# Jiawei-Yang/Denoising-ViT

Measured on AMD Instinct MI355X. Metric: stage-1 images denoised/sec (DINOv2-B/14, 518px, 1k Adam steps), higher is better.
Workload: dtype bf16

## Files before the change

### denoising-vit_amd/csrc/dvt_vit.hip

```cpp
#include <math.h>

#include <type_traits>

#include "../../include/dvt_vit.h"
#include "dvt_common.h"
#include "dvt_ln_row.h"

typedef short bf16x8 __attribute__((ext_vector_type(8)));
typedef short bf16x4 __attribute__((ext_vector_type(4)));
typedef float f32x4 __attribute__((ext_vector_type(4)));
typedef unsigned short bf16_t;

extern int g_f32x3_exact_attention, g_f32x3_unfused;

namespace {

typedef __bf16 hw_bf16x2 __attribute__((ext_vector_type(2)));
typedef float f32x2 __attribute__((ext_vector_type(2)));

__device__ __forceinline__ uint32_t pack2(float a, float b) {
  const hw_bf16x2 v = __builtin_convertvector((f32x2){a, b}, hw_bf16x2);
  return __builtin_bit_cast(uint32_t, v);
}
__device__ __forceinline__ bf16_t f2bf(float f) { return (bf16_t)(pack2(f, 0.f) & 0xffffu); }

constexpr int GBM = 128, GBN = 128, GBK = 64;
int g_vit_gemm_variant = 4;
constexpr int STAGE_BYTES = (GBM + GBN) * GBK * 2;

enum { EPI_BIAS = 0, EPI_QKV = 1, EPI_GELU = 2, EPI_RESID = 3, EPI_EMBED = 4, EPI_F32 = 5, EPI_GELU_X3 = 6, EPI_QKV_X3 = 7,
       EPI_SWIGLU = 8 };
#define IS_QKV(E) ((E) == EPI_QKV || (E) == EPI_QKV_X3)
#define IS_GELU(E) ((E) == EPI_GELU || (E) == EPI_GELU_X3)
#define IS_X3(E) ((E) == EPI_GELU_X3 || (E) == EPI_QKV_X3)

#include "dvt_tile_map.h"

enum { EPOL_RESID_LD = 1,
       EPOL_RESID_ST = 2,
       EPOL_XB_ST = 4,
       EPOL_HID_ST = 8,
       EPOL_QKV_ST = 16,
       EPOL_HID_SC1 = 32,
       EPOL_RESID_SC1 = 64,
       EPOL_ALL = 127,
       EPOL_DEFAULT = EPOL_RESID_LD | EPOL_RESID_ST | EPOL_XB_ST | EPOL_HID_ST | EPOL_HID_SC1 };

struct GemmBArgs {
  const bf16_t* A;
  const bf16_t* W;
  int M, N, K;
  const float* bias;
  bf16_t* out;
  bf16_t* vt;
  bf16_t* out_lo;
  bf16_t* vt_lo;
  float* x;
  const float* gamma;
  const float* pos;
  const float* cls;
  int dim, heads, s_pad, n_tokens;
  int n_prefix, pos_has_cls;
  int group;
  int mblock;
  int nt_store;
  const float2* ln_stats;
  const float* ln_cs;
  bf16_t* xb;
  float2* st_part;
// ... 982 lines not shown
  }
}

#ifdef DVT_LAB
#include "lab/dvt_vit_gemm8t.inc"
#endif
#undef P8B_TILE
#undef P8_STAGE
#undef P8_STAGE_RS
#undef P8_RSRC
#undef P8_RD
#undef P8_LANE_SETUP

#ifdef DVT_LAB
typedef const __attribute__((address_space(4))) GemmBArgs* kernarg_ptr_t;

#include "lab/dvt_vit_gemm4w.inc"
#include "lab/dvt_vit_gemm8p_lab.inc"
#include "lab/dvt_vit_lab.inc"
#endif

int g_vit_group_bytes = 4800 * 1024;
int g_vit_mblock = 0;
int g_vit_nt_store = 0;
int g_vit_xcols = 0;
int g_vit_xcols_bytes = 2400 * 1024;
int g_vit_epi_policy = -1;
int g_vit_fuse_ln = 1;
int g_vit_attn_mask = 15;
int g_vit_stagger_pct = 0;
int g_vit_attn_log2q = 1;
constexpr float ATT_Q_PRESCALE = 0.125f * 1.4426950408889634f;
int g_vit_pf_next = 0;
constexpr int ATT_L2_VAR = 559;
#ifdef DVT_LAB
int g_vit_tpw = 0;
int g_vit_attn_l2_mask = ATT_L2_VAR;
int g_vit_epi_abl = 0;
int g_vit_attn_variant = 2;
int g_vit_abl4w = 0;
int g_vit_8p_build = 0;
unsigned* g_vit_dbg = nullptr;
int g_vit_w4_grid = 0;
#endif

template <int EPI>
int launch_gemm(const GemmBArgs& a0, hipStream_t s) {
  if (a0.M % GBM || a0.N % GBN || a0.K % GBK || a0.M <= 0) return DVT_E_BADARG;
  if (IS_X3(EPI) && a0.M % 256) return DVT_E_BADARG;
  GemmBArgs a = a0;
  if (!a.lda) a.lda = a.K;
  if (!a.ldw) a.ldw = a.K;
  a.dim_ok_sq = (!IS_QKV(EPI)) || (a.dim % 256 == 0);
  if (IS_QKV(EPI) && (a.s_pad <= 0 || a.s_pad % 8 || a.vt_rows <= 0 || a.vt_rows % a.s_pad || a.vt_rows > a.M))
    return DVT_E_BADARG;
  bool sq = g_vit_gemm_variant >= 4;
#ifdef DVT_LAB
  sq = sq || g_vit_gemm_variant == 0;
#endif
  sq = sq && a.M % 256 == 0 && a.N % 256 == 0 && a.dim_ok_sq && a.K >= 2 * GBK && (a.K / GBK) % 2 == 0;
  if (a.ln_stats != nullptr && !(sq || (a.M % G2_BM == 0 && g_vit_gemm_variant != 1))) return DVT_E_BADARG;
  if ((a.xb != nullptr || a.st_part != nullptr) && !(sq && EPI == EPI_RESID && a.xb != nullptr && a.st_part != nullptr))
    return DVT_E_BADARG;
  {
    const int nt = a.N / GBN;
    int g = g_vit_group_bytes / (GBN * a.K * 2);
    g = g < 1 ? 1 : (g > nt ? nt : g);
// ... 260 lines not shown
  const int bb = row / n_tokens, s = row - bb * n_tokens;
  float* y;
  if (s < n_prefix) {
    if (prefix == nullptr) return;
    y = prefix + ((size_t)bb * n_prefix + s) * dim;
  } else {
    y = feat + ((size_t)bb * (n_tokens - n_prefix) + (s - n_prefix)) * dim;
  }
  const float4* xr = reinterpret_cast<const float4*>(x + ((size_t)bb * s_pad + s) * dim);
  const int nq = dim >> 2;
  if (NORM) {
    float4 v[NV];
    float mean, rstd;
    ln_row_stats<NV>(xr, nq, dim, eps, lane, v, mean, rstd);
#pragma unroll
    for (int i = 0; i < NV; ++i) {
      const int q = lane + 64 * i;
      if (q < nq)
        reinterpret_cast<float4*>(y)[q] =
            ln_row_piece(v[i], mean, rstd, reinterpret_cast<const float4*>(w)[q], reinterpret_cast<const float4*>(b)[q]);
    }
  } else {
#pragma unroll
    for (int i = 0; i < NV; ++i) {
      const int q = lane + 64 * i;
      if (q < nq) reinterpret_cast<float4*>(y)[q] = xr[q];
    }
  }
}

__device__ __forceinline__ float max3f(float a, float b, float c) {
  return __builtin_fmaxf(__builtin_fmaxf(a, b), c);
}

constexpr int KV_TILE = 64;
constexpr int VT_LD = 128;

constexpr int ATT_Q = 128;

#ifdef DVT_LAB
#include "lab/dvt_vit_lab_attn.inc"
#endif


constexpr int ATT2_KBUF = 3;

template <int VAR, bool X3>
__device__ __forceinline__ void attention_v2_body(const bf16_t* __restrict__ qk, const bf16_t* __restrict__ vt,
                                                  bf16_t* __restrict__ out, int heads, int s_pad, int n_valid,
                                                  const bf16_t* __restrict__ qk_lo, const bf16_t* __restrict__ vt_lo,
                                                  int split_out = 0) {
  constexpr int NV = (VAR & 64) ? 3 : 2;
  constexpr bool L2D = (VAR & 32) != 0;
  constexpr bool SKIPW = L2D && !(VAR & 128), HALFT = L2D && !(VAR & 256);
  static_assert(!L2D || ((VAR & 4) && !X3 && !(VAR & 64)), "log2-domain build: on the no-max-tree structure, bf16 only");
  constexpr int KBUF = L2D ? 4 : ATT2_KBUF;
  constexpr int KSET = KBUF * KV_TILE * 128, VSET = NV * 64 * VT_LD;
  __shared__ __attribute__((aligned(16))) char smem[(X3 ? 2 : 1) * (KSET + VSET)];
  char* const Kb = smem;
  char* const Vb = smem + KSET;
  char* const Kbl = smem + KSET + VSET;
  char* const Vbl = Kbl + KSET;
  const int tid = threadIdx.x, lane = tid & 63, wave = tid >> 6;
  const int g = lane >> 4, lc = lane & 15;
  const int nqb = (s_pad + ATT_Q - 1) / ATT_Q;
  int id = blockIdx.x;
  {
    const int nwg = gridDim.x, q = nwg >> 3, r = nwg & 7, xcd = id & 7, loc = id >> 3;
    id = (xcd < r ? xcd * (q + 1) : r * (q + 1) + (xcd - r) * q) + loc;
  }
  const int qb = id % nqb, h = (id / nqb) % heads, b = id / (nqb * heads);
  const int dim = heads * 64, ldq = 2 * dim;
  const size_t row0 = (size_t)b * s_pad;

  bf16x8 qf[2], qfl[2];
  auto load_q = [&](const bf16_t* base, bf16x8 (&dst)[2]) {
    const bf16_t* qrow = base + (row0 + qb * ATT_Q + wave * 16 + lc) * ldq + h * 64;
#pragma unroll
    for (int ks = 0; ks < 2; ++ks) {
      union { bf16x8 v; uint32_t u[4]; } raw;
      raw.v = *reinterpret_cast<const bf16x8*>(qrow + ks * 32 + g * 8);
      if constexpr (!L2D) {
#pragma unroll
        for (int j = 0; j < 4; ++j) {
          const float lo = __uint_as_float(raw.u[j] << 16) * 0.125f;
          const float hi = __uint_as_float(raw.u[j] & 0xffff0000u) * 0.125f;
          raw.u[j] = pack2(lo, hi);
        }
      }
      dst[ks] = raw.v;
    }
  };
  load_q(qk, qf);
  if constexpr (X3) load_q(qk_lo, qfl);
  const bf16_t* kbase = qk + row0 * ldq + dim + h * 64;
  const bf16_t* vbase = vt + ((size_t)(b * heads + h) * 64) * s_pad;

  f32x4 o[4];
#pragma unroll
  for (int i = 0; i < 4; ++i) o[i] = (f32x4){0.f, 0.f, 0.f, 0.f};
  float m_run = L2D ? 0.f : -1e30f, l_run = 0.f;
  f32x4 cinit = (f32x4){0.f, 0.f, 0.f, 0.f};
  const f32x4 zero4 = (f32x4){0.f, 0.f, 0.f, 0.f};
  const bool active = !SKIPW || qb * ATT_Q + __builtin_amdgcn_readfirstlane(wave) * 16 < s_pad;
  const float LOG2E = 1.4426950408889634f;
  const float THR = 8.0f;

  const int ntiles = (n_valid + KV_TILE - 1) / KV_TILE;
  const int sr0 = tid >> 3, sc = tid & 7;
  const bf16_t* kp0 = kbase + (size_t)sr0 * ldq + sc * 8;
  const bf16_t* vp0 = vbase + (size_t)sr0 * s_pad + sc * 8;
  const int kdo = sr0 * 128 + ((sc ^ (sr0 & 7)) << 4);
  const int vks = sc >> 2, vc = sc & 3, vsw = (sr0 >> 1) & 7;
  const int vdo0 = sr0 * VT_LD + (((vks * 4 + 2 * (vc & 1)) ^ vsw) << 4) + (vc >> 1) * 8;
  const int vdo1 = sr0 * VT_LD + (((vks * 4 + 2 * (vc & 1) + 1) ^ vsw) << 4) + (vc >> 1) * 8;
  uint4 kr0, vr0, kr0l, vr0l;
  const ptrdiff_t klo = X3 ? (qk_lo - qk) : 0, vlo = X3 ? (vt_lo - vt) : 0;
  const unsigned klane = (unsigned)(sr0 * ldq + sc * 8) * 2u;
  const unsigned vlane = (unsigned)(sr0 * s_pad + sc * 8) * 2u, vlane0 = (unsigned)(sr0 * s_pad) * 2u;
#define A2_LOADK(kt)                                                                                 \
  do {                                                                                               \
    if constexpr (L2D) {                                                                             \
      kr0 = *reinterpret_cast<const uint4*>(reinterpret_cast<const char*>(kbase + (size_t)(kt) * KV_TILE * ldq) + klane); \
    } else {                                                                                         \
      kr0 = *reinterpret_cast<const uint4*>(kp0 + (size_t)(kt) * KV_TILE * ldq);                     \
    }                                                                                                \
    if constexpr (X3) kr0l = *reinterpret_cast<const uint4*>(kp0 + klo + (size_t)(kt) * KV_TILE * ldq); \
  } while (0)
#define A2_LOADV(kt)                                                                   \
  do {                                                                                 \
    if constexpr (L2D) {                                                               \
      const unsigned vo_ = (kt) * KV_TILE + sc * 8 >= s_pad ? vlane0 : vlane;          \
      vr0 = *reinterpret_cast<const uint4*>(reinterpret_cast<const char*>(vbase + (kt) * KV_TILE) + vo_); \
    } else {                                                                           \
      const int vk_ = (kt) * KV_TILE + sc * 8 >= s_pad ? -sc * 8 : (kt) * KV_TILE;     \
      vr0 = *reinterpret_cast<const uint4*>(vp0 + vk_);                                \
      if constexpr (X3) vr0l = *reinterpret_cast<const uint4*>(vp0 + vlo + vk_);       \
    }                                                                                  \
  } while (0)
#define A2_STOREK(kt)                                                                                   \
  do {                                                                                                  \
    *reinterpret_cast<uint4*>(Kb + ((kt) % KBUF) * (KV_TILE * 128) + kdo) = kr0;                   \
    if constexpr (X3) *reinterpret_cast<uint4*>(Kbl + ((kt) % KBUF) * (KV_TILE * 128) + kdo) = kr0l; \
  } while (0)
#define A2_STOREV(kt)                                                                     \
  do {                                                                                    \
    char* vb_ = Vb + ((kt) % NV) * (64 * VT_LD);                                          \
    *reinterpret_cast<uint2*>(vb_ + vdo0) = make_uint2(vr0.x, vr0.y);                     \
    *reinterpret_cast<uint2*>(vb_ + vdo1) = make_uint2(vr0.z, vr0.w);                     \
    if constexpr (X3) {                                                                   \
      char* vl_ = Vbl + ((kt) % NV) * (64 * VT_LD);                                       \
      *reinterpret_cast<uint2*>(vl_ + vdo0) = make_uint2(vr0l.x, vr0l.y);                 \
// ... 11 lines not shown
          const int krow = mt * 16 + lc, ko_ = krow * 128 + (((ks * 4 + g) ^ (krow & 7)) << 4);                     \
          kh_[mt] = *reinterpret_cast<const bf16x8*>(Ks_ + ko_);                                                   \
          kl_[mt] = *reinterpret_cast<const bf16x8*>(Kl_ + ko_);                                                   \
          if (ks == 0) dst[mt] = (f32x4){0.f, 0.f, 0.f, 0.f};                                                      \
        }                                                                                                          \
        _Pragma("unroll") for (int mt = 0; mt < 4; ++mt)                                                           \
          dst[mt] = __builtin_amdgcn_mfma_f32_16x16x32_bf16(kl_[mt], qf[ks], dst[mt], 0, 0, 0);                    \
        _Pragma("unroll") for (int mt = 0; mt < 4; ++mt)                                                           \
          dst[mt] = __builtin_amdgcn_mfma_f32_16x16x32_bf16(kh_[mt], qfl[ks], dst[mt], 0, 0, 0);                   \
        _Pragma("unroll") for (int mt = 0; mt < 4; ++mt)                                                           \
          dst[mt] = __builtin_amdgcn_mfma_f32_16x16x32_bf16(kh_[mt], qf[ks], dst[mt], 0, 0, 0);                    \
      }                                                                                                            \
    } else if constexpr (VAR & 1) {                                                                                       \
      _Pragma("unroll") for (int ks = 0; ks < 2; ++ks) {                                                           \
        _Pragma("unroll") for (int mt = 0; mt < 4; ++mt) {                                                         \
          const int krow = mt * 16 + lc;                                                                           \
          const bf16x8 kf = *reinterpret_cast<const bf16x8*>(Ks_ + krow * 128 + (((ks * 4 + g) ^ (krow & 7)) << 4)); \
          if (ks == 0) dst[mt] = L2D ? cinit : zero4;                                                              \
          dst[mt] = __builtin_amdgcn_mfma_f32_16x16x32_bf16(kf, qf[ks], dst[mt], 0, 0, 0);                         \
        }                                                                                                          \
      }                                                                                                            \
    } else {                                                                                                       \
    _Pragma("unroll") for (int mt = 0; mt < 4; ++mt) {                                                             \
      dst[mt] = L2D ? cinit : zero4;                                                                               \
      _Pragma("unroll") for (int ks = 0; ks < 2; ++ks) {                                                           \
        const int krow = mt * 16 + lc;                                                                             \
        const bf16x8 kf = *reinterpret_cast<const bf16x8*>(Ks_ + krow * 128 + (((ks * 4 + g) ^ (krow & 7)) << 4)); \
        dst[mt] = __builtin_amdgcn_mfma_f32_16x16x32_bf16(kf, qf[ks], dst[mt], 0, 0, 0);                           \
      }                                                                                                            \
    }                                                                                                              \
    }                                                                                                              \
  } while (0)

  A2_LOADK(0);
  A2_LOADV(0);
  A2_STOREK(0);
  A2_STOREV(0);
  if constexpr (L2D) {
    const int last = ntiles - 1;
    A2_LOADK(1 < last ? 1 : last);
    A2_STOREK(1);
    A2_LOADK(2 < last ? 2 : last);
    A2_LOADV(1 < last ? 1 : last);
  } else {
    if (ntiles > 1) {
      A2_LOADK(1);
      A2_STOREK(1);
    }
    if (ntiles > 2) A2_LOADK(2);
    if (ntiles > 1) A2_LOADV(1);
  }
  __syncthreads();
  f32x4 sA[4], sB[4];
  auto lane_quad_max = [&](float v) {
    const unsigned u = __float_as_uint(v);
    const auto r16 = __builtin_amdgcn_permlane16_swap(u, u, false, false);
    v = fmaxf(__uint_as_float(r16[0]), __uint_as_float(r16[1]));
    const unsigned u2 = __float_as_uint(v);
    const auto r32 = __builtin_amdgcn_permlane32_swap(u2, u2, false, false);
    return fmaxf(__uint_as_float(r32[0]), __uint_as_float(r32[1]));
  };
  auto max16 = [&](const f32x4 (&s)[4]) {
    float tmax = __builtin_fmaxf(__builtin_fmaxf(s[0][0], s[0][1]), s[0][2]);
    tmax = max3f(tmax, s[0][3], s[1][0]);
    tmax = max3f(tmax, s[1][1], s[1][2]);
    tmax = max3f(tmax, s[1][3], s[2][0]);
    tmax = max3f(tmax, s[2][1], s[2][2]);
    tmax = max3f(tmax, s[2][3], s[3][0]);
    tmax = max3f(tmax, s[3][1], s[3][2]);
    return fmaxf(tmax, s[3][3]);
  };
  if (active) A2_S(sA, 0);
  if constexpr (L2D) {
    if (active) {
      if (n_valid < KV_TILE) {
#pragma unroll
        for (int mt = 0; mt < 4; ++mt)
#pragma unroll
          for (int r = 0; r < 4; ++r)
            if (mt * 16 + 4 * g + r >= n_valid) sA[mt][r] = -1e30f;
      }
      m_run = lane_quad_max(max16(sA));
      cinit = (f32x4){-m_run, -m_run, -m_run, -m_run};
#pragma unroll
      for (int mt = 0; mt < 4; ++mt) sA[mt] += cinit;
    }
  }
  if constexpr (VAR & 16) {
    if (wave >= 4) __builtin_amdgcn_s_setprio(1);
  }
  if constexpr (VAR & 64) {
    if (wave >= 4) __syncthreads();
  }
  union PF { bf16x8 v; uint32_t u[4]; };
  auto tile = [&](int kt, auto last_tag, f32x4 (&s)[4], f32x4 (&sn)[4]) {
    constexpr bool LAST = decltype(last_tag)::value;
    if constexpr (L2D) {
      const int last = ntiles - 1;
      A2_STOREK(kt + 2);
      A2_STOREV(kt + 1);
      if constexpr (!LAST) {
        const int k3 = kt + 3 < last ? kt + 3 : last, v2 = kt + 2 < last ? kt + 2 : last;
        A2_LOADK(k3);
        A2_LOADV(v2);
      }
    } else {
    if (kt + 2 < ntiles) A2_STOREK(kt + 2);
    if (kt + 1 < ntiles) A2_STOREV(kt + 1);
    if (kt + 3 < ntiles) A2_LOADK(kt + 3);
    if (kt + 2 < ntiles) A2_LOADV(kt + 2);
    }
    if constexpr (LAST) {
      const int kbase_idx = kt * KV_TILE;
#pragma unroll
      for (int mt = 0; mt < 4; ++mt)
#pragma unroll
        for (int r = 0; r < 4; ++r)
          if (kbase_idx + mt * 16 + 4 * g + r >= n_valid) s[mt][r] = -1e30f;
    }
    auto exact_max = [&]() {
      if constexpr (L2D) {
        const float d = fmaxf(lane_quad_max(max16(s)), 0.f);
        const float alpha = __builtin_amdgcn_exp2f(-d);
        l_run *= alpha;
#pragma unroll
        for (int i = 0; i < 4; ++i) o[i] *= alpha;
        m_run += d;
        cinit = (f32x4){-m_run, -m_run, -m_run, -m_run};
        const f32x4 d4 = {d, d, d, d};
#pragma unroll
        for (int mt = 0; mt < 4; ++mt) {
          s[mt] -= d4;
          if constexpr (!LAST) sn[mt] -= d4;
        }
        return;
      }
// ... 35 lines not shown
      if (!__all(tmax <= m_run + THR)) {
        const unsigned u = __float_as_uint(tmax);
        const auto r16 = __builtin_amdgcn_permlane16_swap(u, u, false, false);
        tmax = fmaxf(__uint_as_float(r16[0]), __uint_as_float(r16[1]));
        const unsigned u2 = __float_as_uint(tmax);
        const auto r32 = __builtin_amdgcn_permlane32_swap(u2, u2, false, false);
        tmax = fmaxf(__uint_as_float(r32[0]), __uint_as_float(r32[1]));
        const float m_new = fmaxf(m_run, tmax);
        const float alpha = __builtin_amdgcn_exp2f((m_run - m_new) * LOG2E);
        l_run *= alpha;
#pragma unroll
        for (int i = 0; i < 4; ++i) {
          o[i][0] *= alpha;
          o[i][1] *= alpha;
          o[i][2] *= alpha;
          o[i][3] *= alpha;
        }
        m_run = m_new;
      }
    }
    if constexpr (HALFT && LAST) {
      if (n_valid - kt * KV_TILE <= 32) {
        float hp[2][4];
        f32x2 hs2;
        auto half_softmax = [&]() {
          hs2 = (f32x2){0.f, 0.f};
#pragma unroll
          for (int mt = 0; mt < 2; ++mt)
#pragma unroll
            for (int h2 = 0; h2 < 2; ++h2) {
              f32x2 e;
              e.x = __builtin_amdgcn_exp2f(s[mt][2 * h2]);
              e.y = __builtin_amdgcn_exp2f(s[mt][2 * h2 + 1]);
              hs2 += e;
              hp[mt][2 * h2] = e.x;
              hp[mt][2 * h2 + 1] = e.y;
            }
        };
        half_softmax();
        float hsum = hs2.x + hs2.y;
        if (!__all(hsum <= 2980.0f)) {
          exact_max();
          half_softmax();
          hsum = hs2.x + hs2.y;
        }
        l_run += hsum;
        union { bf16x8 v; uint32_t u[4]; } hf;
        hf.u[0] = pack2(hp[0][0], hp[0][1]); hf.u[1] = pack2(hp[0][2], hp[0][3]);
        hf.u[2] = pack2(hp[1][0], hp[1][1]); hf.u[3] = pack2(hp[1][2], hp[1][3]);
        const char* Vh = Vb + (kt % NV) * (64 * VT_LD);
#pragma unroll
        for (int mt = 0; mt < 4; ++mt) {
          const int vr = mt * 16 + lc, vs_ = (vr >> 1) & 7;
          const bf16x8 vf = *reinterpret_cast<const bf16x8*>(Vh + vr * VT_LD + ((g ^ vs_) << 4));
          o[mt] = __builtin_amdgcn_mfma_f32_16x16x32_bf16(vf, hf.v, o[mt], 0, 0, 0);
        }
        __syncthreads();
        return;
      }
    }
    if constexpr (L2D && !LAST && (VAR & 16384)) {
      union PH { bf16x8 v; uint32_t u[4]; };
      float hp[4][4];
      auto soft_half = [&](int h) {
        f32x2 a2, b2;
#pragma unroll
        for (int q = 0; q < 2; ++q) {
          const int mt = 2 * h + q;
          f32x2 e0, e1;
          e0.x = __builtin_amdgcn_exp2f(s[mt][0]);
          e0.y = __builtin_amdgcn_exp2f(s[mt][1]);
          e1.x = __builtin_amdgcn_exp2f(s[mt][2]);
          e1.y = __builtin_amdgcn_exp2f(s[mt][3]);
          if (q == 0) {
            a2 = e0;
            b2 = e1;
          } else {
            a2 += e0;
            b2 += e1;
          }
          hp[mt][0] = e0.x; hp[mt][1] = e0.y; hp[mt][2] = e1.x; hp[mt][3] = e1.y;
        }
        a2 += b2;
        return a2.x + a2.y;
      };
      auto pack_half = [&](int h, PH& f) {
        f.u[0] = pack2(hp[2 * h][0], hp[2 * h][1]); f.u[1] = pack2(hp[2 * h][2], hp[2 * h][3]);
        f.u[2] = pack2(hp[2 * h + 1][0], hp[2 * h + 1][1]); f.u[3] = pack2(hp[2 * h + 1][2], hp[2 * h + 1][3]);
      };
      PH f0, f1;
      __builtin_amdgcn_sched_barrier(0);
      A2_S(sn, kt + 1);
      float ps = soft_half(0);
      pack_half(0, f0);
      __builtin_amdgcn_sched_group_barrier(0x100, 4, 0);
#pragma unroll
      for (int i = 0; i < 8; ++i) {
        __builtin_amdgcn_sched_group_barrier(0x002, 2, 0);
        __builtin_amdgcn_sched_group_barrier(0x008, 1, 0);
        if (i < 4) __builtin_amdgcn_sched_group_barrier(0x100, 1, 0);
      }
      __builtin_amdgcn_sched_barrier(0);
      if (!__all(ps <= 2980.0f)) {
        exact_max();
        ps = soft_half(0);
        pack_half(0, f0);
      }
      l_run += ps;
      const char* Vs2 = Vb + (kt % NV) * (64 * VT_LD);
      bf16x8 vf[8];
#pragma unroll
      for (int mt = 0; mt < 4; ++mt) {
        const int vr = mt * 16 + lc, vs_ = (vr >> 1) & 7;
        const char* vrow = Vs2 + vr * VT_LD;
        vf[mt] = *reinterpret_cast<const bf16x8*>(vrow + ((g ^ vs_) << 4));
        vf[4 + mt] = *reinterpret_cast<const bf16x8*>(vrow + (((4 + g) ^ vs_) << 4));
      }
#pragma unroll
      for (int mt = 0; mt < 4; ++mt) o[mt] = __builtin_amdgcn_mfma_f32_16x16x32_bf16(vf[mt], f0.v, o[mt], 0, 0, 0);
      float ps1 = soft_half(1);
      pack_half(1, f1);
      __builtin_amdgcn_sched_group_barrier(0x100, 8, 0);
#pragma unroll
      for (int i = 0; i < 4; ++i) {
        __builtin_amdgcn_sched_group_barrier(0x008, 1, 0);
        __builtin_amdgcn_sched_group_barrier(0x002, 4, 0);
      }
      __builtin_amdgcn_sched_barrier(0);
      if (!__all(ps1 <= 2980.0f)) {
        exact_max();
        ps1 = soft_half(1);
        pack_half(1, f1);
      }
      l_run += ps1;
#pragma unroll
      for (int mt = 0; mt < 4; ++mt) o[mt] = __builtin_amdgcn_mfma_f32_16x16x32_bf16(vf[4 + mt], f1.v, o[mt], 0, 0, 0);
      __syncthreads();
      return;
    }
    __builtin_amdgcn_sched_barrier(0);
    if constexpr (VAR & 4096) __builtin_amdgcn_s_setprio(1);
    if constexpr (!LAST) A2_S(sn, kt + 1);
    const f32x2 l2e2 = {LOG2E, LOG2E};
    float pv[4][4];
    f32x2 ps2;
    auto softmax = [&]() {
      const float mb = m_run * LOG2E;
      const f32x2 nmb2 = {-mb, -mb};
      f32x2 psb;
      if constexpr (!L2D) ps2 = (f32x2){0.f, 0.f};
#pragma unroll
      for (int mt = 0; mt < 4; ++mt)
#pragma unroll
        for (int h2 = 0; h2 < 2; ++h2) {
          const f32x2 sv = {s[mt][2 * h2], s[mt][2 * h2 + 1]};
          const f32x2 t = L2D ? sv : __builtin_elementwise_fma(sv, l2e2, nmb2);
          f32x2 e;
          e.x = __builtin_amdgcn_exp2f(t.x);
          e.y = __builtin_amdgcn_exp2f(t.y);
          if constexpr (L2D) {
            if (mt == 0) (h2 == 0 ? ps2 : psb) = e;
            else (h2 == 0 ? ps2 : psb) += e;
          } else {
            ps2 += e;
          }
          pv[mt][2 * h2] = e.x;
          pv[mt][2 * h2 + 1] = e.y;
        }
      if constexpr (L2D) ps2 += psb;
    };
    softmax();
    float psum = ps2.x + ps2.y;
    PF pf0, pf1, pl0, pl1;
    auto pack = [&]() {
      pf0.u[0] = pack2(pv[0][0], pv[0][1]); pf0.u[1] = pack2(pv[0][2], pv[0][3]);
      pf0.u[2] = pack2(pv[1][0], pv[1][1]); pf0.u[3] = pack2(pv[1][2], pv[1][3]);
      pf1.u[0] = pack2(pv[2][0], pv[2][1]); pf1.u[1] = pack2(pv[2][2], pv[2][3]);
      pf1.u[2] = pack2(pv[3][0], pv[3][1]); pf1.u[3] = pack2(pv[3][2], pv[3][3]);
      if constexpr (X3) {
        auto lo2 = [](uint32_t hb, float a, float b) {
          return pack2(a - __uint_as_float(hb << 16), b - __uint_as_float(hb & 0xffff0000u));
        };
        pl0.u[0] = lo2(pf0.u[0], pv[0][0], pv[0][1]); pl0.u[1] = lo2(pf0.u[1], pv[0][2], pv[0][3]);
        pl0.u[2] = lo2(pf0.u[2], pv[1][0], pv[1][1]); pl0.u[3] = lo2(pf0.u[3], pv[1][2], pv[1][3]);
        pl1.u[0] = lo2(pf1.u[0], pv[2][0], pv[2][1]); pl1.u[1] = lo2(pf1.u[1], pv[2][2], pv[2][3]);
        pl1.u[2] = lo2(pf1.u[2], pv[3][0], pv[3][1]); pl1.u[3] = lo2(pf1.u[3], pv[3][2], pv[3][3]);
      }
    };
    if constexpr (!(VAR & 1024)) pack();
    if constexpr (!LAST && (VAR & 32768)) {
      __builtin_amdgcn_iglp_opt((VAR & 65536) ? 3 : 2);
    } else if constexpr (!LAST && (VAR & 512)) {
      __builtin_amdgcn_sched_group_barrier(0x100, 4, 0);
#pragma unroll
      for (int i = 0; i < 8; ++i) {
        __builtin_amdgcn_sched_group_barrier(0x002, 4, 0);
        __builtin_amdgcn_sched_group_barrier(0x008, 1, 0);
        if (i < 4) __builtin_amdgcn_sched_group_barrier(0x100, 1, 0);
      }
    } else if constexpr (!LAST) {
#pragma unroll
      for (int i = 0; i < (X3 ? 24 : 8); ++i) {
        __builtin_amdgcn_sched_group_barrier(0x008, 1, 0);
        __builtin_amdgcn_sched_group_barrier(0x002, (X3 || L2D) ? 4 : (VAR & 4) ? 5 : 6, 0);
      }
    }
    __builtin_amdgcn_sched_barrier(0);
    if constexpr (VAR & 4096) __builtin_amdgcn_s_setprio(0);
    if constexpr (VAR & 4) {
      if (!__all(psum <= 2980.0f)) {
        exact_max();
        softmax();
        psum = ps2.x + ps2.y;
        if constexpr (!(VAR & 1024)) pack();
      }
    }
    l_run += psum;
    if constexpr (VAR & 64) __syncthreads();
    const char* Vs = Vb + (kt % NV) * (64 * VT_LD);
    if constexpr (X3) {
      const char* Vl = Vbl + (kt % NV) * (64 * VT_LD);
#pragma unroll
      for (int mt = 0; mt < 4; ++mt) {
        const int vr = mt * 16 + lc, vs_ = (vr >> 1) & 7;
        const int o0_ = vr * VT_LD + ((g ^ vs_) << 4), o1_ = vr * VT_LD + (((4 + g) ^ vs_) << 4);
        const bf16x8 vh0 = *reinterpret_cast<const bf16x8*>(Vs + o0_), vh1 = *reinterpret_cast<const bf16x8*>(Vs + o1_);
        const bf16x8 vl0 = *reinterpret_cast<const bf16x8*>(Vl + o0_), vl1 = *reinterpret_cast<const bf16x8*>(Vl + o1_);
        o[mt] = __builtin_amdgcn_mfma_f32_16x16x32_bf16(vl0, pf0.v, o[mt], 0, 0, 0);
        o[mt] = __builtin_amdgcn_mfma_f32_16x16x32_bf16(vl1, pf1.v, o[mt], 0, 0, 0);
        o[mt] = __builtin_amdgcn_mfma_f32_16x16x32_bf16(vh0, pl0.v, o[mt], 0, 0, 0);
        o[mt] = __builtin_amdgcn_mfma_f32_16x16x32_bf16(vh1, pl1.v, o[mt], 0, 0, 0);
        o[mt] = __builtin_amdgcn_mfma_f32_16x16x32_bf16(vh0, pf0.v, o[mt], 0, 0, 0);
        o[mt] = __builtin_amdgcn_mfma_f32_16x16x32_bf16(vh1, pf1.v, o[mt], 0, 0, 0);
      }
    } else if constexpr (VAR & 2) {
      if constexpr (VAR & 2048) __builtin_amdgcn_s_setprio(1);
      bf16x8 vf[8];
#pragma unroll
      for (int mt = 0; mt < 4; ++mt) {
        const int vr = mt * 16 + lc, vs_ = (vr >> 1) & 7;
        const char* vrow = Vs + vr * VT_LD;
        vf[mt] = *reinterpret_cast<const bf16x8*>(vrow + ((g ^ vs_) << 4));
        vf[4 + mt] = *reinterpret_cast<const bf16x8*>(vrow + (((4 + g) ^ vs_) << 4));
      }
      if constexpr (VAR & 1024) pack();
#pragma unroll
      for (int mt = 0; mt < 4; ++mt) o[mt] = __builtin_amdgcn_mfma_f32_16x16x32_bf16(vf[mt], pf0.v, o[mt], 0, 0, 0);
#pragma unroll
      for (int mt = 0; mt < 4; ++mt) o[mt] = __builtin_amdgcn_mfma_f32_16x16x32_bf16(vf[4 + mt], pf1.v, o[mt], 0, 0, 0);
      __builtin_amdgcn_sched_group_barrier(0x100, 8, 0);
      if constexpr (VAR & 1024) __builtin_amdgcn_sched_group_barrier(0x002, 8, 0);
      __builtin_amdgcn_sched_group_barrier(0x008, 8, 0);
      if constexpr (VAR & 2048) __builtin_amdgcn_s_setprio(0);
    } else {
#pragma unroll
      for (int mt = 0; mt < 4; ++mt) {
        const int vr = mt * 16 + lc, vs_ = (vr >> 1) & 7;
        const char* vrow = Vs + vr * VT_LD;
        const bf16x8 vf0 = *reinterpret_cast<const bf16x8*>(vrow + ((g ^ vs_) << 4));
        const bf16x8 vf1 = *reinterpret_cast<const bf16x8*>(vrow + (((4 + g) ^ vs_) << 4));
        o[mt] = __builtin_amdgcn_mfma_f32_16x16x32_bf16(vf0, pf0.v, o[mt], 0, 0, 0);
        o[mt] = __builtin_amdgcn_mfma_f32_16x16x32_bf16(vf1, pf1.v, o[mt], 0, 0, 0);
      }
    }
    if constexpr (VAR & 8192) {
      asm volatile("s_waitcnt lgkmcnt(0)" ::: "memory");
    } else {
      __syncthreads();
    }
  };
  if constexpr (SKIPW) {
    if (!active) {
      const int last = ntiles - 1;
      for (int kt = 0; kt < ntiles; ++kt) {
        A2_STOREK(kt + 2);
        A2_STOREV(kt + 1);
        A2_LOADK(kt + 3 < last ? kt + 3 : last);
        A2_LOADV(kt + 2 < last ? kt + 2 : last);
        __syncthreads();
      }
      return;
    }
  }
  if constexpr (L2D) {
    int kt = 0;
    for (; kt + 4 <= ntiles - 1; kt += 4) {
      tile(kt, std::false_type{}, sA, sB);
      tile(kt + 1, std::false_type{}, sB, sA);
      tile(kt + 2, std::false_type{}, sA, sB);
      tile(kt + 3, std::false_type{}, sB, sA);
    }
    for (; kt < ntiles - 1; ++kt) {
      tile(kt, std::false_type{}, sA, sB);
#pragma unroll
      for (int mt = 0; mt < 4; ++mt) sA[mt] = sB[mt];
    }
    tile(ntiles - 1, std::true_type{}, sA, sB);
  } else if constexpr (VAR & 8) {
    int kt = 0;
    for (; kt + 2 <= ntiles - 1; kt += 2) {
      tile(kt, std::false_type{}, sA, sB);
      tile(kt + 1, std::false_type{}, sB, sA);
    }
    if (kt < ntiles - 1) {
      tile(kt, std::false_type{}, sA, sB);
      tile(ntiles - 1, std::true_type{}, sB, sA);
    } else {
      tile(ntiles - 1, std::true_type{}, sA, sB);
    }
  } else {
    for (int kt = 0; kt < ntiles - 1; ++kt) {
      tile(kt, std::false_type{}, sA, sB);
#pragma unroll
      for (int mt = 0; mt < 4; ++mt) sA[mt] = sB[mt];
    }
    tile(ntiles - 1, std::true_type{}, sA, sB);
  }
  if constexpr (VAR & 16) __builtin_amdgcn_s_setprio(0);
  if constexpr (VAR & 64) {
    if (wave < 4) __syncthreads();
  }
#undef A2_LOADK
#undef A2_LOADV
#undef A2_STOREK
#undef A2_STOREV
#undef A2_S
  if (qb * ATT_Q + wave * 16 >= s_pad) return;
  l_run += __shfl_xor(l_run, 16, 64);
  l_run += __shfl_xor(l_run, 32, 64);
  const float inv = 1.0f / l_run;
  if constexpr (X3) {
    if (split_out) {
      bf16_t* r3 = out + (row0 + qb * ATT_Q + wave * 16 + lc) * (3 * dim) + h * 64;
#pragma unroll
      for (int mt = 0; mt < 4; ++mt) {
        const float a0 = o[mt][0] * inv, a1 = o[mt][1] * inv, a2 = o[mt][2] * inv, a3 = o[mt][3] * inv;
        uint2 hh, ll;
        hh.x = pack2(a0, a1);
        hh.y = pack2(a2, a3);
        ll.x = pack2(a0 - __uint_as_float(hh.x << 16), a1 - __uint_as_float(hh.x & 0xffff0000u));
        ll.y = pack2(a2 - __uint_as_float(hh.y << 16), a3 - __uint_as_float(hh.y & 0xffff0000u));
        bf16_t* c = r3 + mt * 16 + 4 * g;
        *reinterpret_cast<uint2*>(c) = hh;
        *reinterpret_cast<uint2*>(c + dim) = hh;
        *reinterpret_cast<uint2*>(c + 2 * dim) = ll;
      }
      return;
    }
    float* orow = reinterpret_cast<float*>(out) + (row0 + qb * ATT_Q + wave * 16 + lc) * dim + h * 64;
#pragma unroll
    for (int mt = 0; mt < 4; ++mt)
      *reinterpret_cast<float4*>(orow + mt * 16 + 4 * g) =
          make_float4(o[mt][0] * inv, o[mt][1] * inv, o[mt][2] * inv, o[mt][3] * inv);
    return;
  }
// ... 113 lines not shown
    return 0;
  }
  if (v <= -200000 && v >= -200000 - EPOL_ALL) {
    const int rs = (-200000 - v) & 7;
    if (rs == 3 || rs == 5 || rs == 6) return DVT_E_BADARG;
    g_vit_epi_policy = -200000 - v;
    return 0;
  }
  if (v <= -570 && v >= -572) {
    g_vit_pf_next = -570 - v;
    return 0;
  }
  if (v == -530 || v == -531) {
    g_vit_attn_log2q = v == -531;
    return 0;
  }
  if (v == -520 || v == -521) {
    g_f32x3_exact_attention = v == -520;
    return 0;
  }
  if (v == -522 || v == -523) {
    g_f32x3_unfused = v == -522;
    return 0;
  }
#ifdef DVT_LAB
  if ((v <= -600 && v > -700) || (v < -1100 && v >= -1100 - 65536)) {
    g_vit_w4_grid = v > -700 ? -600 - v : -1100 - v;
    return 0;
  }
  if (v <= -560 && v >= -563) {
    g_vit_epi_abl = -560 - v;
    return 0;
  }
  if (v == -540 || v == -540 - 2 || v == -540 - 128 || v == -540 - 256 || v == -540 - 384 || v == -540 - 512 || v == -540 - 514 || v == -540 - 1024 || v == -540 - 2048 || v == -540 - 4096 || v == -540 - 8192 || v == -540 - 16384 || v == -540 - 32768 || v == -540 - 32768 - 65536) {
    g_vit_attn_l2_mask = ATT_L2_VAR ^ (-540 - v);
    return 0;
  }
  if (v <= -510 && v > -530) {
    g_vit_attn_mask = -510 - v;
    return 0;
  }
  if (v == -510 - 31 || v == -510 - 64 || v == -510 - 79) {
    g_vit_attn_mask = -510 - v;
    return 0;
  }
  if (v == -501 || v == -502) {
    g_vit_attn_variant = -500 - v;
    return 0;
  }
  if (v <= -300 && v > -399) {
    const int n = -300 - v;
    g_vit_abl4w = g_vit_8p_build = 0;
    if (n == 0) return 0;
    if (g_vit_gemm_variant >= 6 && g_vit_gemm_variant <= 9) g_vit_abl4w = n;
    else if (g_vit_gemm_variant == 5 && (n == 3 || (n >= 6 && n <= 9))) g_vit_8p_build = n;
    else return DVT_E_BADARG;
    return 0;
  }
  if (v <= -200 && v > -300) {
    g_vit_tpw = -200 - v > 64 ? 64 : -200 - v;
    return 0;
  }
#else
  if (v == -502 || v == -510 - 15) return 0;
#endif
  if (v <= -700 && v >= -1100) {
    g_vit_stagger_pct = -700 - v;
// ... 250 lines not shown

extern "C" int dvt_vit_layernorm(const float* x, const float* w, const float* b, void* y, int rows,
                                 int dim, float eps, void* stream) {
  if (!x || !w || !b || !y || rows < 0 || dim <= 0 || dim % 4 || dim > 1536) return DVT_E_BADARG;
  if (rows == 0) return 0;
  if (dim <= 1024)
    hipLaunchKernelGGL((layernorm_kernel<false, 4>), dim3(dvt_cdiv(rows, 4)), dim3(256), 0,
                       (hipStream_t)stream, x, w, b, (bf16_t*)y, (float*)nullptr, rows, dim, eps, 0, 0, 0);
  else
    hipLaunchKernelGGL((layernorm_kernel<false, 6>), dim3(dvt_cdiv(rows, 4)), dim3(256), 0,
                       (hipStream_t)stream, x, w, b, (bf16_t*)y, (float*)nullptr, rows, dim, eps, 0, 0, 0);
  DVT_CHECK_LAUNCH();
  return 0;
}

extern "C" int dvt_vit_attention_log2q(const void* qk, const void* vt, void* out, int batch, int heads,
                                       int s_pad, int n_valid, void* stream) {
  if (!qk || !vt || !out || batch <= 0 || heads <= 0 || s_pad % 16 || n_valid <= 0 || n_valid > s_pad)
    return DVT_E_BADARG;
  DvtProbeScope probe(DVT_PROBE_VIT_ATTN, (hipStream_t)stream,
                      4.0 * (double)n_valid * n_valid * 64.0 * heads * batch);
  const dim3 grid(((s_pad + ATT_Q - 1) / ATT_Q) * heads * batch);
#ifdef DVT_LAB
  if (g_vit_attn_l2_mask != ATT_L2_VAR) {
#define A2L_VAR(n)                                                                                                    \
  if (g_vit_attn_l2_mask == (n)) {                                                                                    \
    hipLaunchKernelGGL(attention_kernel_l2<(n)>, grid, dim3(512), 0, (hipStream_t)stream, (const bf16_t*)qk,          \
                       (const bf16_t*)vt, (bf16_t*)out, heads, s_pad, n_valid);                                       \
    DVT_CHECK_LAUNCH();                                                                                               \
    return 0;                                                                                                         \
  }
    A2L_VAR(ATT_L2_VAR ^ 2) A2L_VAR(ATT_L2_VAR ^ 128) A2L_VAR(ATT_L2_VAR ^ 256) A2L_VAR(ATT_L2_VAR ^ 384) A2L_VAR(ATT_L2_VAR ^ 512)
    A2L_VAR(ATT_L2_VAR ^ 514) A2L_VAR(ATT_L2_VAR ^ 1024) A2L_VAR(ATT_L2_VAR ^ 2048) A2L_VAR(ATT_L2_VAR ^ 4096) A2L_VAR(ATT_L2_VAR ^ 8192) A2L_VAR(ATT_L2_VAR ^ 16384) A2L_VAR(ATT_L2_VAR ^ 32768) A2L_VAR(ATT_L2_VAR ^ (32768 + 65536))
#undef A2L_VAR
    return DVT_E_BADARG;
  }
#endif
  hipLaunchKernelGGL(attention_kernel_l2<ATT_L2_VAR>, grid, dim3(512), 0, (hipStream_t)stream, (const bf16_t*)qk,
                     (const bf16_t*)vt, (bf16_t*)out, heads, s_pad, n_valid);
  DVT_CHECK_LAUNCH();
  return 0;
}

extern "C" int dvt_vit_attention(const void* qk, const void* vt, void* out, int batch, int heads,
                                 int s_pad, int n_valid, void* stream) {
  if (!qk || !vt || !out || batch <= 0 || heads <= 0 || s_pad % 16 || n_valid <= 0 || n_valid > s_pad)
    return DVT_E_BADARG;
  DvtProbeScope probe(DVT_PROBE_VIT_ATTN, (hipStream_t)stream,
                      4.0 * (double)n_valid * n_valid * 64.0 * heads * batch);
  const dim3 grid(((s_pad + ATT_Q - 1) / ATT_Q) * heads * batch);
#ifdef DVT_LAB
  if (g_vit_attn_variant != 2) {
    if (s_pad % ATT_Q) return DVT_E_BADARG;
    hipLaunchKernelGGL(attention_kernel, grid, dim3(512), 0, (hipStream_t)stream, (const bf16_t*)qk, (const bf16_t*)vt,
                       (bf16_t*)out, heads, s_pad, n_valid);
    DVT_CHECK_LAUNCH();
    return 0;
  }
  bool done = false;
#define A2_VAR(n)                                                                                                     \
  if (g_vit_attn_mask == n) {                                                                                         \
    hipLaunchKernelGGL(attention_kernel_v2<n>, grid, dim3(512), 0, (hipStream_t)stream, (const bf16_t*)qk,            \
                       (const bf16_t*)vt, (bf16_t*)out, heads, s_pad, n_valid);                                       \
    done = true;                                                                                                      \
  }
  A2_VAR(0) A2_VAR(1) A2_VAR(2) A2_VAR(4) A2_VAR(8) A2_VAR(16) A2_VAR(64) A2_VAR(3) A2_VAR(15) A2_VAR(31) A2_VAR(79)
// ... 273 lines not shown
```

Before: 3.054.

## Stage attention K tiles via buffer-load-to-LDS DMA and restructure softmax sums

The default log2-domain attention build turns on three new options. K tiles now go straight from global memory into LDS with buffer_load...lds, replacing the register load-then-store path. The softmax row sum on the hot path becomes a split-chain tree reduction, held in place by opaque asm barriers. A new round-8 sched_group_barrier pattern interleaves MFMA with VALU and LDS ops. The aim is to cut VGPR pressure and LDS-store instructions and to shorten dependency chains, at the cost of changed wait/vmcnt synchronization and a different summation order.

```diff
diff --git a/denoising-vit_amd/csrc/dvt_attn_stage_map.h b/denoising-vit_amd/csrc/dvt_attn_stage_map.h
--- /dev/null
+++ b/denoising-vit_amd/csrc/dvt_attn_stage_map.h
@@ -0,0 +1,41 @@
+#pragma once
+
+#if defined(__HIPCC__)
+#define DVT_ASM_FN __host__ __device__ __forceinline__
+#else
+#define DVT_ASM_FN inline
+#endif
+
+constexpr int ATT_K_ROW_BYTES = 128;
+constexpr int ATT_K_TILE_ROWS = 64;
+constexpr int ATT_K_BUF_BYTES = ATT_K_TILE_ROWS * ATT_K_ROW_BYTES;
+constexpr int ATT_K_WAVE_BYTES = 64 * 16;
+
+struct AttKStage {
+  int row;
+  int chunk;
+  int lds_off;
+};
+
+DVT_ASM_FN AttKStage att_k_stage_reg(int tid) {
+  AttKStage s;
+  s.row = tid >> 3;
+  s.chunk = tid & 7;
+  s.lds_off = s.row * ATT_K_ROW_BYTES + ((s.chunk ^ (s.row & 7)) << 4);
+  return s;
+}
+
+DVT_ASM_FN AttKStage att_k_stage_dma(int tid) {
+  AttKStage s;
+  const int wave = tid >> 6, lane = tid & 63;
+  s.lds_off = wave * ATT_K_WAVE_BYTES + lane * 16;
+  s.row = s.lds_off / ATT_K_ROW_BYTES;
+  s.chunk = ((s.lds_off >> 4) & 7) ^ (s.row & 7);
+  return s;
+}
+
+DVT_ASM_FN unsigned att_k_src_bytes(const AttKStage& s, int ldq) { return (unsigned)(s.row * ldq + s.chunk * 8) * 2u; }
+
+DVT_ASM_FN unsigned att_k_records(int ntiles, int ldq) {
+  return (unsigned)(ntiles * ATT_K_TILE_ROWS - 1) * (unsigned)ldq * 2u + (unsigned)ATT_K_ROW_BYTES;
+}
diff --git a/denoising-vit_amd/csrc/dvt_vit.hip b/denoising-vit_amd/csrc/dvt_vit.hip
--- a/denoising-vit_amd/csrc/dvt_vit.hip
+++ b/denoising-vit_amd/csrc/dvt_vit.hip
@@ -35,6 +35,7 @@
 #define IS_X3(E) ((E) == EPI_GELU_X3 || (E) == EPI_QKV_X3)
 
 #include "dvt_tile_map.h"
+#include "dvt_attn_stage_map.h"
 
 enum { EPOL_RESID_LD = 1,
        EPOL_RESID_ST = 2,
@@ -1083,7 +1084,7 @@
 int g_vit_attn_log2q = 1;
 constexpr float ATT_Q_PRESCALE = 0.125f * 1.4426950408889634f;
 int g_vit_pf_next = 0;
-constexpr int ATT_L2_VAR = 559;
+constexpr int ATT_L2_VAR = 559 + 7340032;
 #ifdef DVT_LAB
 int g_vit_tpw = 0;
 int g_vit_attn_l2_mask = ATT_L2_VAR;
@@ -1410,6 +1411,10 @@
 __device__ __forceinline__ float max3f(float a, float b, float c) {
   return __builtin_fmaxf(__builtin_fmaxf(a, b), c);
 }
+__device__ __forceinline__ float opaque_f32(float x) {
+  asm("" : "+v"(x));
+  return x;
+}
 
 constexpr int KV_TILE = 64;
 constexpr int VT_LD = 128;
@@ -1431,7 +1436,9 @@
   constexpr int NV = (VAR & 64) ? 3 : 2;
   constexpr bool L2D = (VAR & 32) != 0;
   constexpr bool SKIPW = L2D && !(VAR & 128), HALFT = L2D && !(VAR & 256);
+  constexpr bool SADD = L2D && (VAR & 1048576), KDMA = L2D && (VAR & 2097152), RD8 = L2D && (VAR & 4194304);
   static_assert(!L2D || ((VAR & 4) && !X3 && !(VAR & 64)), "log2-domain build: on the no-max-tree structure, bf16 only");
+  static_assert(L2D || !(VAR & (1048576 + 2097152 + 4194304)), "round-8 levers: log2-domain builds only");
   constexpr int KBUF = L2D ? 4 : ATT2_KBUF;
   constexpr int KSET = KBUF * KV_TILE * 128, VSET = NV * 64 * VT_LD;
   __shared__ __attribute__((aligned(16))) char smem[(X3 ? 2 : 1) * (KSET + VSET)];
@@ -1488,7 +1495,7 @@
   const int sr0 = tid >> 3, sc = tid & 7;
   const bf16_t* kp0 = kbase + (size_t)sr0 * ldq + sc * 8;
   const bf16_t* vp0 = vbase + (size_t)sr0 * s_pad + sc * 8;
-  const int kdo = sr0 * 128 + ((sc ^ (sr0 & 7)) << 4);
+  const int kdo = att_k_stage_reg(tid).lds_off;
   const int vks = sc >> 2, vc = sc & 3, vsw = (sr0 >> 1) & 7;
   const int vdo0 = sr0 * VT_LD + (((vks * 4 + 2 * (vc & 1)) ^ vsw) << 4) + (vc >> 1) * 8;
   const int vdo1 = sr0 * VT_LD + (((vks * 4 + 2 * (vc & 1) + 1) ^ vsw) << 4) + (vc >> 1) * 8;
@@ -1496,6 +1503,16 @@
   const ptrdiff_t klo = X3 ? (qk_lo - qk) : 0, vlo = X3 ? (vt_lo - vt) : 0;
   const unsigned klane = (unsigned)(sr0 * ldq + sc * 8) * 2u;
   const unsigned vlane = (unsigned)(sr0 * s_pad + sc * 8) * 2u, vlane0 = (unsigned)(sr0 * s_pad) * 2u;
+  const unsigned kdlane = att_k_src_bytes(att_k_stage_dma(tid), ldq);
+  const auto krs = __builtin_amdgcn_make_buffer_rsrc((void*)kbase, 0, KDMA ? att_k_records(ntiles, ldq) : 0u, 0x00020000);
+  char* const kdw = Kb + __builtin_amdgcn_readfirstlane(wave) * ATT_K_WAVE_BYTES;
+#define A2_KWAIT()                                \
+  do {                                            \
+    if constexpr (KDMA) wait_vm<0>();             \
+  } while (0)
+#define A2_DMAK(kb, kt)                      \
+  __builtin_amdgcn_raw_ptr_buffer_load_lds(krs, (lds_ptr_t)(kdw + ((kb) % KBUF) * ATT_K_BUF_BYTES), 16, kdlane, \
+                                           (kt) * (KV_TILE * ldq * 2), 0, 0)
 #define A2_LOADK(kt)                                                                                 \
   do {                                                                                               \
     if constexpr (L2D) {                                                                             \
@@ -1573,11 +1590,23 @@
     }                                                                                                              \
   } while (0)
 
+  if constexpr (KDMA) {
+    const int last = ntiles - 1;
+    A2_DMAK(0, 0);
+    A2_DMAK(1, 1 < last ? 1 : last);
+    A2_LOADV(0);
+    A2_STOREV(0);
+    A2_KWAIT();
+    A2_DMAK(2, 2 < last ? 2 : last);
+    A2_LOADV(1 < last ? 1 : last);
+  } else {
   A2_LOADK(0);
   A2_LOADV(0);
   A2_STOREK(0);
   A2_STOREV(0);
-  if constexpr (L2D) {
+  }
+  if constexpr (KDMA) {
+  } else if constexpr (L2D) {
     const int last = ntiles - 1;
     A2_LOADK(1 < last ? 1 : last);
     A2_STOREK(1);
@@ -1638,11 +1667,13 @@
     constexpr bool LAST = decltype(last_tag)::value;
     if constexpr (L2D) {
       const int last = ntiles - 1;
-      A2_STOREK(kt + 2);
+      if constexpr (KDMA) A2_KWAIT();
+      else A2_STOREK(kt + 2);
       A2_STOREV(kt + 1);
       if constexpr (!LAST) {
         const int k3 = kt + 3 < last ? kt + 3 : last, v2 = kt + 2 < last ? kt + 2 : last;
-        A2_LOADK(k3);
+        if constexpr (KDMA) A2_DMAK(kt + 3, k3);
+        else A2_LOADK(k3);
         A2_LOADV(v2);
       }
     } else {
@@ -1744,7 +1775,12 @@
               f32x2 e;
               e.x = __builtin_amdgcn_exp2f(s[mt][2 * h2]);
               e.y = __builtin_amdgcn_exp2f(s[mt][2 * h2 + 1]);
-              hs2 += e;
+              if constexpr (SADD) {
+                hs2.x = opaque_f32(hs2.x + e.x);
+                hs2.y = opaque_f32(hs2.y + e.y);
+              } else {
+                hs2 += e;
+              }
               hp[mt][2 * h2] = e.x;
               hp[mt][2 * h2 + 1] = e.y;
             }
@@ -1787,13 +1823,21 @@
           if (q == 0) {
             a2 = e0;
             b2 = e1;
+          } else if constexpr (SADD) {
+            a2.x = opaque_f32(a2.x + e0.x); a2.y = opaque_f32(a2.y + e0.y);
+            b2.x = opaque_f32(b2.x + e1.x); b2.y = opaque_f32(b2.y + e1.y);
           } else {
             a2 += e0;
             b2 += e1;
           }
           hp[mt][0] = e0.x; hp[mt][1] = e0.y; hp[mt][2] = e1.x; hp[mt][3] = e1.y;
         }
-        a2 += b2;
+        if constexpr (SADD) {
+          a2.x = opaque_f32(a2.x + b2.x);
+          a2.y = opaque_f32(a2.y + b2.y);
+        } else {
+          a2 += b2;
+        }
         return a2.x + a2.y;
       };
       auto pack_half = [&](int h, PH& f) {
@@ -1856,10 +1900,24 @@
     const f32x2 l2e2 = {LOG2E, LOG2E};
     float pv[4][4];
     f32x2 ps2;
-    auto softmax = [&]() {
+    float pss = 0.f;
+    auto softmax = [&](auto hot_tag) {
       const float mb = m_run * LOG2E;
       const f32x2 nmb2 = {-mb, -mb};
       f32x2 psb;
+      if constexpr (SADD && decltype(hot_tag)::value) {
+        float ch[4];
+#pragma unroll
+        for (int mt = 0; mt < 4; ++mt)
+#pragma unroll
+          for (int r = 0; r < 4; ++r) {
+            const float e = __builtin_amdgcn_exp2f(s[mt][r]);
+            pv[mt][r] = e;
+            ch[r] = mt == 0 ? e : (ch[r] + e);
+          }
+        pss = opaque_f32(opaque_f32(ch[0]) + opaque_f32(ch[2])) + opaque_f32(opaque_f32(ch[1]) + opaque_f32(ch[3]));
+        return;
+      }
       if constexpr (!L2D) ps2 = (f32x2){0.f, 0.f};
 #pragma unroll
       for (int mt = 0; mt < 4; ++mt)
@@ -1881,8 +1939,8 @@
         }
       if constexpr (L2D) ps2 += psb;
     };
-    softmax();
-    float psum = ps2.x + ps2.y;
+    softmax(std::true_type{});
+    float psum = SADD ? pss : ps2.x + ps2.y;
     PF pf0, pf1, pl0, pl1;
     auto pack = [&]() {
       pf0.u[0] = pack2(pv[0][0], pv[0][1]); pf0.u[1] = pack2(pv[0][2], pv[0][3]);
@@ -1902,11 +1960,18 @@
     if constexpr (!(VAR & 1024)) pack();
     if constexpr (!LAST && (VAR & 32768)) {
       __builtin_amdgcn_iglp_opt((VAR & 65536) ? 3 : 2);
+    } else if constexpr (!LAST && RD8) {
+#pragma unroll
+      for (int i = 0; i < 8; ++i) {
+        if (i == 0) __builtin_amdgcn_sched_group_barrier(0x100, 8, 0);
+        __builtin_amdgcn_sched_group_barrier(0x002, SADD ? 5 : 4, 0);
+        __builtin_amdgcn_sched_group_barrier(0x008, 1, 0);
+      }
     } else if constexpr (!LAST && (VAR & 512)) {
       __builtin_amdgcn_sched_group_barrier(0x100, 4, 0);
 #pragma unroll
       for (int i = 0; i < 8; ++i) {
-        __builtin_amdgcn_sched_group_barrier(0x002, 4, 0);
+        __builtin_amdgcn_sched_group_barrier(0x002, SADD ? 5 : 4, 0);
         __builtin_amdgcn_sched_group_barrier(0x008, 1, 0);
         if (i < 4) __builtin_amdgcn_sched_group_barrier(0x100, 1, 0);
       }
@@ -1920,9 +1985,10 @@
     __builtin_amdgcn_sched_barrier(0);
     if constexpr (VAR & 4096) __builtin_amdgcn_s_setprio(0);
     if constexpr (VAR & 4) {
-      if (!__all(psum <= 2980.0f)) {
+      const bool grew = !__all(psum <= 2980.0f);
+      if (SADD ? __builtin_expect(grew, 0) : grew) {
         exact_max();
-        softmax();
+        softmax(std::false_type{});
         psum = ps2.x + ps2.y;
         if constexpr (!(VAR & 1024)) pack();
       }
@@ -1985,12 +2051,15 @@
     if (!active) {
       const int last = ntiles - 1;
       for (int kt = 0; kt < ntiles; ++kt) {
-        A2_STOREK(kt + 2);
+        if constexpr (KDMA) A2_KWAIT();
+        else A2_STOREK(kt + 2);
         A2_STOREV(kt + 1);
-        A2_LOADK(kt + 3 < last ? kt + 3 : last);
+        if constexpr (KDMA) A2_DMAK(kt + 3, kt + 3 < last ? kt + 3 : last);
+        else A2_LOADK(kt + 3 < last ? kt + 3 : last);
         A2_LOADV(kt + 2 < last ? kt + 2 : last);
         __syncthreads();
       }
+      A2_KWAIT();
       return;
     }
   }
@@ -2033,6 +2102,8 @@
     if (wave < 4) __syncthreads();
   }
 #undef A2_LOADK
+#undef A2_DMAK
+#undef A2_KWAIT
 #undef A2_LOADV
 #undef A2_STOREK
 #undef A2_STOREV
@@ -2212,7 +2283,8 @@
     g_vit_epi_abl = -560 - v;
     return 0;
   }
-  if (v == -540 || v == -540 - 2 || v == -540 - 128 || v == -540 - 256 || v == -540 - 384 || v == -540 - 512 || v == -540 - 514 || v == -540 - 1024 || v == -540 - 2048 || v == -540 - 4096 || v == -540 - 8192 || v == -540 - 16384 || v == -540 - 32768 || v == -540 - 32768 - 65536) {
+  if (v == -540 || v == -540 - 2 || v == -540 - 128 || v == -540 - 256 || v == -540 - 384 || v == -540 - 512 || v == -540 - 514 || v == -540 - 1024 || v == -540 - 2048 || v == -540 - 4096 || v == -540 - 8192 || v == -540 - 16384 || v == -540 - 32768 || v == -540 - 32768 - 65536 ||
+      ((-540 - v) > 0 && ((-540 - v) & ~(1048576 + 2097152 + 4194304)) == 0)) {
     g_vit_attn_l2_mask = ATT_L2_VAR ^ (-540 - v);
     return 0;
   }
@@ -2529,6 +2601,8 @@
   }
     A2L_VAR(ATT_L2_VAR ^ 2) A2L_VAR(ATT_L2_VAR ^ 128) A2L_VAR(ATT_L2_VAR ^ 256) A2L_VAR(ATT_L2_VAR ^ 384) A2L_VAR(ATT_L2_VAR ^ 512)
     A2L_VAR(ATT_L2_VAR ^ 514) A2L_VAR(ATT_L2_VAR ^ 1024) A2L_VAR(ATT_L2_VAR ^ 2048) A2L_VAR(ATT_L2_VAR ^ 4096) A2L_VAR(ATT_L2_VAR ^ 8192) A2L_VAR(ATT_L2_VAR ^ 16384) A2L_VAR(ATT_L2_VAR ^ 32768) A2L_VAR(ATT_L2_VAR ^ (32768 + 65536))
+    A2L_VAR(ATT_L2_VAR ^ 1048576) A2L_VAR(ATT_L2_VAR ^ 2097152) A2L_VAR(ATT_L2_VAR ^ 4194304) A2L_VAR(ATT_L2_VAR ^ 3145728)
+    A2L_VAR(ATT_L2_VAR ^ 6291456) A2L_VAR(ATT_L2_VAR ^ 5242880) A2L_VAR(ATT_L2_VAR ^ 7340032)
 #undef A2L_VAR
     return DVT_E_BADARG;
   }
```

Measured after the change: 3.079, median of 6. About the same (+0.8%).
